# JiuTongBro/vqnerf_release

Measured on AMD Instinct MI355X. Metric: rays/sec (render) 800x800, 64+64 samples/ray, NeuS SDF 8x256 + colour 4x256, higher is better.
Workload: dtype f32; 1 GPU; BASELINE configs[1], nerf/hotdog-shaped NeuS render: one whole 800x800 pin-hole view per rank per step (camera at distance 4, fov 0.6911), n_samples=64, n_importance=64, up_sample_steps=4, sdf 8x256; parallelism=views x1 (no data-path collective)

## Files before the change

include/vqn_neus_fold.h:

```cpp
#ifndef VQN_NEUS_FOLD_H_
#define VQN_NEUS_FOLD_H_
#include <stdint.h>
#ifdef __cplusplus
extern "C" {
#endif

int64_t vqn_neus_fold_pack(const int32_t* sdf_desc, const int32_t* col_desc, const float* wbuf_col, int64_t col_floats,
                           const float* sdf_w_last, const float* sdf_b_last, int sdf_hidden, int d_feature, const float* col_w0,
                           const float* col_b0, int col_hidden, float* wbuf_out, int64_t out_floats, int32_t* col_desc_out,
                           void* stream);

int vqn_mc_classify(const float* u, int nx, int ny, int nz, float threshold, int32_t* vert_count, int32_t* tri_count, void* stream);
int vqn_mc_emit(const float* u, int nx, int ny, int nz, float threshold, const int32_t* vert_offset, const int32_t* tri_offset,
                int64_t n_verts, int64_t n_tris, const float* origin, const float* step, float* verts, int32_t* tris, void* stream);

int vqn_mesh_components(const int32_t* tris, int64_t n_tris, int64_t n_verts, int32_t* labels, void* stream);
int vqn_mesh_remap_tris(const int32_t* tris_in, int64_t n_tris, const uint8_t* keep_tri, const int32_t* tri_offset,
                        const int32_t* new_index, int64_t n_verts, int32_t* tris_out, int64_t n_out, void* stream);

int vqn_mc_brick_points(const float* ax, const float* ay, const float* az, int nx, int ny, int nz, const int32_t* brick_ijk,
                        int64_t n_bricks, int64_t first, int64_t count, float* pts, void* stream);
int vqn_mc_brick_classify(const float* ub, const int32_t* brick_ijk, int64_t n_bricks, const int32_t* slot, int nx, int ny, int nz,
                          float threshold, int32_t* vert_count, int32_t* tri_count, int64_t* keys, int32_t* leaks, void* stream);
int vqn_mc_brick_emit(const float* ub, const int32_t* brick_ijk, int64_t n_bricks, const int32_t* slot, int nx, int ny, int nz,
                      float threshold, const int32_t* vert_offset, const int32_t* tri_offset, int64_t n_verts, int64_t n_tris,
                      const float* origin, const float* step, float* verts, int32_t* tris, void* stream);

int64_t vqn_image_metrics_scratch_bytes(int64_t B, int H, int W);
int vqn_image_metrics_u8(const uint8_t* a, const uint8_t* b, const float* alpha, int64_t alpha_stride, float alpha_thres, int64_t B,
                         int H, int W, int C, const double* window, void* scratch, int64_t scratch_bytes, void* out, void* stream);
int vqn_image_metrics_f32(const float* a, const float* b, const float* alpha, int64_t alpha_stride, float alpha_thres, int64_t B,
                          int H, int W, int C, const double* window, void* scratch, int64_t scratch_bytes, void* out, void* stream);

int64_t vqn_seg_scratch_bytes(int64_t n, int R, int C);
int vqn_seg_contingency_rgb(const uint8_t* gt_rgb, const uint8_t* pd_rgb, const float* alpha, float alpha_thres, int64_t n,
                            const uint8_t* gt_palette, int n_gt, const uint8_t* pd_palette, int n_pd, void* scratch,
                            int64_t scratch_bytes, void* out, void* stream);
int vqn_seg_contingency_labels(const int32_t* gt, const int32_t* pd, const uint8_t* mask, int64_t n, int n_gt, int n_pd,
                               void* scratch, int64_t scratch_bytes, void* out, void* stream);

int vqn_meanshift_seek(const double* points, int64_t n, const double* seeds, int64_t n_seeds, int D, double bandwidth, int max_iter,
                       double* means, int32_t* counts, int32_t* iters, void* stream);
int64_t vqn_meanshift_merge_scratch_bytes(int64_t n_candidates, int D);
int vqn_meanshift_merge(const double* candidates, const int32_t* cand_counts, int64_t n_candidates, int D, double bandwidth,
                        void* scratch, int64_t scratch_bytes, uint8_t* kept, int32_t* n_kept, void* stream);
int vqn_meanshift_assign(const double* points, int64_t n, const double* centres, int K, int D, double bandwidth, int32_t* labels,
                         double* dist, void* stream);

#ifdef __cplusplus
}
#endif
#endif
```

vqnerf_release_amd/_C.py:

```python
import contextlib
import ctypes
import os
import re

import numpy as np
import torch

_HERE = os.path.dirname(os.path.abspath(__file__))
LIB_PATH = os.environ.get('VQN_LIB', os.path.join(_HERE, 'lib', 'libvqnerf_hip.so'))
_lib = None

_ABI = """
i vqn_version()  s vqn_last_error()  i vqn_vq_assign(plipipppppp)  i vqn_vq_assign_variant(iiii)  i vqn_vq_ema_stats(ppliippplp)
l vqn_vq_ema_stats_ws_bytes(lii)  i vqn_vq_ste_loss(pplfpppp)  i vqn_vq_ema_update(pppiidfpppppppp)
i vqn_decomp_loss_fwd(ppppppliiffffffpp)  i vqn_decomp_loss_bwd(ppppppliiffffffpppppp)  i vqn_l2_normalize_rows(plifpp)
i vqn_l2_normalize_rows_bwd(pplifpp)  i vqn_vq_ste_loss_bwd(pppplpp)  i vqn_codebook_prep(ppiifpp)  i vqn_sim_smooth_fwd(piifpp)
i vqn_sim_smooth_bwd(pppiifpp)  i vqn_vq_quantize_rows(plipipffpppppp)  i vqn_vq_train_bwd(pppppflifpp)
i vqn_vq_quantize_rows_train(plipipfffppppppp)  i vqn_mlp_chain_fwd(ppplpipipipip)  i vqn_mlp_chain_fwd_f16s(ppplpipipipip)
i vqn_brdf_shade_fwd(pppppppliippppppppppppipipp)  i vqn_brdf_shade_fwd_rows(ppppppppliippppppppppppipipp)
l vqn_brdf_shade_bwd_partials(l)  i vqn_brdf_shade_bwd(pppppppliipppppppppppppppp)  i vqn_neus_sdf_points(pppppplipp)
l vqn_neus_fine_scratch_bytes(p)  i vqn_neus_fine_points(pppppppppliplpppp)  i vqn_neus_train_fwd(pppppplplpiiiipppp)
l vqn_neus_train_bwd_scratch_bytes(p)  i vqn_neus_train_bwd(ppppppplplpipip)  l vqn_neus_train_bwd_x3_scratch_bytes(p)
i vqn_neus_train_bwd_x3(pppppppplplpipip)  i vqn_pack_x3_gather(pplpp)  i vqn_pack_x3_gather2(pplpplpp)
i vqn_neus_sdf_points_f16s(pppppplipp)  i vqn_neus_fine_points_f16s(pppppppppliplpppp)  i vqn_neus_sdf_points_x3(pppppplipp)
i vqn_neus_fine_points_x3(pppppppppliplpppp)  i vqn_neus_train_fwd_x3(pppppplplpiiiipppp)  i vqn_neus_pack_create(piiifiiiiiip)
i vqn_neus_pack_update(pppppp)  p vqn_neus_pack_sdf_desc(p)  p vqn_neus_pack_col_desc(p)  p vqn_neus_pack_sdf_wbuf(p)
p vqn_neus_pack_col_wbuf(p)  l vqn_neus_pack_sdf_floats(p)  l vqn_neus_pack_col_floats(p)  v vqn_neus_pack_destroy(p)
l vqn_neus_sdf_pack_plan(piiifiiippl)  l vqn_neus_col_pack_plan(iiiiiiiiippl)  i vqn_mlp_chain_vq_fwd(ppppplpppppiffpppppp)
i vqn_vq_codebook_frags(piipp)  i vqn_linear2srgb(plpp)  i vqn_chain_pack_create(iiiipp)  i vqn_chain_pack_update(pppp)
i vqn_chain_pack_n_weights(p)  p vqn_chain_pack_desc(p)  p vqn_chain_pack_wbuf(p)  l vqn_chain_pack_floats(p)
v vqn_chain_pack_destroy(p)  l vqn_chain_pack_plan(iiiipppl)  i vqn_neus_upsample(ppppliffpipp)  i vqn_neus_merge(ppppliippp)
i vqn_neus_section_mids(plifpppp)  i vqn_neus_composite_fwd(pppppppppliffppppppppppp)  i vqn_neus_composite_bwd(pppppppppliffpppppppppp)
i vqn_tile_program(pppppilp)  l vqn_tile_program_grid(pl)  i vqn_weight_norm_fwd(ipppppp)  i vqn_weight_norm_bwd(ipppppppp)
i vqn_tfmt_pack(plilpip)  i vqn_tfmt_pack_delta(plilpipip)  i vqn_tfmt_unpack(piliplp)  i vqn_wgrad_partials(piiipiiilippp)
i vqn_wgrad_partials_x3(piiipiiilippp)  i vqn_wgrad_partials_batched(ipppppppplippip)  i vqn_reduce_partials(piiiplip)
i vqn_wgrad_finalize(ipppppppppppppp)  i vqn_clip_preserve(plffpp)  i vqn_loss_total(plppiiipp)  i vqn_ks_split_fwd(ppilppp)
i vqn_ks_split_bwd(ppilppppp)  i vqn_wgrad_thin_batched(ippppppppplippp)  i vqn_multi_copy(ipppp)  i vqn_refl_train_desc_ints()
i vqn_refl_train_fwd_x3(ppppplpippiip)  i vqn_refl_train_fwd_x3_zx(pppppplpipppiip)  l vqn_refl_train_bwd_x3_scratch_bytes(p)
i vqn_refl_train_bwd_x3(ppplpppipipippiiiplp)  i vqn_adam_step(ippppppppdddddiip)
"""
ABI = {name: (ret, args) for ret, name, args in re.findall(r'(\w) (\w+)\((\w*)\)', _ABI)}
ABI_FOLD = {'vqn_neus_fold_pack': ('l', 'ppplppiippiplpp'), 'vqn_mc_classify': ('i', 'piiifppp'), 'vqn_mc_emit': ('i', 'piiifppllppppp'),
            'vqn_mesh_components': ('i', 'pllpp'), 'vqn_mesh_remap_tris': ('i', 'plppplplp'),
            'vqn_mc_brick_points': ('i', 'pppiiiplllpp'), 'vqn_mc_brick_classify': ('i', 'pplpiiifppppp'),
            'vqn_mc_brick_emit': ('i', 'pplpiiifppllppppp'), 'vqn_image_metrics_scratch_bytes': ('l', 'lii'),
            'vqn_image_metrics_u8': ('i', 'ppplfliiipplpp'), 'vqn_image_metrics_f32': ('i', 'ppplfliiipplpp'),
            'vqn_seg_scratch_bytes': ('l', 'lii'), 'vqn_seg_contingency_rgb': ('i', 'pppflpipiplpp'),
            'vqn_seg_contingency_labels': ('i', 'pppliiplpp'), 'vqn_meanshift_seek': ('i', 'plplidipppp'),
            'vqn_meanshift_merge_scratch_bytes': ('l', 'li'), 'vqn_meanshift_merge': ('i', 'pplidplppp'),
            'vqn_meanshift_assign': ('i', 'plpiidppp')}
_CTYPES = dict(p=ctypes.c_void_p, i=ctypes.c_int, l=ctypes.c_int64, f=ctypes.c_float, d=ctypes.c_double, s=ctypes.c_char_p, v=None)


class VqnError(RuntimeError):
    pass


def build(verbose=False):
    import subprocess
    cmd = ['make', '-C', os.path.join(_HERE, 'csrc'), '-j8']
    if not verbose:
        cmd.append('-s')
    subprocess.check_call(cmd)


def lib():
    global _lib
    if _lib is None:
        if not os.path.exists(LIB_PATH):
            raise VqnError(f'{LIB_PATH} is missing: run `python -c "import __graft_entry__ as g; g.build()"` '
                           '(or `make -C vqnerf_release_amd/csrc`). There is no non-HIP fallback.')
        L = ctypes.CDLL(LIB_PATH)
        for name, (ret, args) in list(ABI.items()) + list(ABI_FOLD.items()):
            f = getattr(L, name)
            f.restype, f.argtypes = _CTYPES[ret], [_CTYPES[a] for a in args]
        _lib = L
    return _lib


def require_device(t, what):
    if not t.is_cuda:
        raise VqnError(f'{what}: got a {t.device} tensor; the no-graph path runs on MI355X HIP kernels only '
                       '(there is no CPU fallback)')
    lib()


def _check(rc, name, count=False):
    if (rc > 0) if count else (rc == 0):
        return rc
    raise VqnError(f'{name} failed (rc={rc or -3}): {lib().vqn_last_error().decode()}')


def _call(name, *args, clock=True, count=False):
    with _clock(name if clock is True else clock) if clock else contextlib.nullcontext():
        rc = getattr(lib(), name)(*args, _stream())
    return _check(rc, name, count)


def _ptr(t):
    return t if t is None or isinstance(t, int) else t.data_ptr()


def _ptrs(ts, n=1):
    return (ctypes.c_void_p * max(n, len(ts)))(*[_ptr(t) for t in ts])


def _host(a, dtype=np.int32):
    return np.ascontiguousarray(a, dtype=dtype).ctypes


def _i32(desc):
    d = np.ascontiguousarray(desc, dtype=np.int32)
    return d, d.ctypes.data_as(ctypes.c_void_p)


def _stream():
    return torch.cuda.current_stream().cuda_stream


class KernelClock:
    enabled = False
    pairs = {}
    _free = []

    @classmethod
# ... 184 lines not shown
    if g_ste is not None:
        _f32c(g_ste, 'g_ste')
    gz = torch.empty_like(z)
    _call('vqn_vq_train_bwd', _ptr(z), _ptr(xnorm), _ptr(quant), _ptr(g_ste), _ptr(g_loss), loss_post, z.shape[0], z.shape[1], eps, _ptr(gz))
    return gz


def l2_normalize_rows(x, eps=1e-6):
    _f32c(x, 'x')
    y = torch.empty_like(x)
    _call('vqn_l2_normalize_rows', _ptr(x), x.shape[0], x.shape[1], eps, _ptr(y))
    return y


def vq_quantize_rows(z, codebook, sel_mask=None, eps=1e-6, want_ste=True, want_xnorm=False, loss_post=1.0):
    _f32c(z, 'z'); _f32c(codebook, 'codebook')
    N, D = z.shape
    K = codebook.shape[1]
    assert codebook.shape[0] == D
    dev = z.device
    idx = torch.empty((N,), dtype=torch.int64, device=dev)
    ste = torch.empty((N, D), dtype=torch.float32, device=dev) if want_ste else None
    loss = torch.empty((), dtype=torch.float32, device=dev)
    counts = torch.empty((K,), dtype=torch.float32, device=dev)
    ws = torch.empty((4096,), dtype=torch.float32, device=dev)
    if sel_mask is not None:
        sel_mask = _f32c(sel_mask.reshape(-1).to(torch.float32).contiguous(), 'sel_mask')
        assert sel_mask.numel() == K
    n = N * D
    if want_xnorm:
        xnorm = torch.empty((N, D), dtype=torch.float32, device=dev)
        _call('vqn_vq_quantize_rows_train', _ptr(z), N, D, _ptr(codebook), K, _ptr(sel_mask), eps, 1.0 / n if n else 0.0, loss_post, _ptr(ws),
              _ptr(idx), _ptr(ste), _ptr(loss), _ptr(counts), _ptr(xnorm))
        return idx, ste, loss, counts, xnorm
    _call('vqn_vq_quantize_rows', _ptr(z), N, D, _ptr(codebook), K, _ptr(sel_mask), eps, 1.0 / n if n else 0.0, _ptr(ws), _ptr(idx), _ptr(ste),
          _ptr(loss), _ptr(counts))
    return idx, ste, loss, counts


_scratch_cache = {}
_scratch_held = []


def _scratch(tag, need, device, stream=None, capturing=None):
    if stream is None:
        stream = torch.cuda.current_stream().cuda_stream
    if capturing is None:
        capturing = torch.cuda.is_current_stream_capturing()
    key = (str(device), stream, tag)
    entry = _scratch_cache.get(key)
    if entry is None or entry[0].numel() < need:
        if entry is not None and entry[1]:
            _scratch_held.append(entry[0])
        entry = _scratch_cache[key] = [torch.empty((need,), dtype=torch.uint8, device=device), False]
    entry[1] = entry[1] or capturing
    return entry[0]


def _scratch_bytes(name, desc):
    need = getattr(lib(), name)(desc)
    if need <= 0:
        raise VqnError(f'{name}: invalid descriptor')
    return need


def neus_sdf_points(sdf_desc, wbuf_sdf, rays_o=None, rays_d=None, z=None, pts=None, mode='f32', pack=None):
    if pack is not None:
        dp, wp = pack.sdf_desc, pack.sdf_wbuf
    else:
        _f32c(wbuf_sdf, 'wbuf_sdf')
        dp, wp = _host(sdf_desc), _ptr(wbuf_sdf)
    if pts is not None:
        _f32c(pts, 'pts'); P, S = pts.shape[0], 1
        dev = pts.device
    else:
        _f32c(rays_o, 'rays_o'); _f32c(rays_d, 'rays_d'); _f32c(z, 'z')
        B, S = z.shape
        P = B * S
        dev = z.device
    out = torch.empty((P,), dtype=torch.float32, device=dev)
    entry = {'f32': 'vqn_neus_sdf_points', 'f16s': 'vqn_neus_sdf_points_f16s', 'x3': 'vqn_neus_sdf_points_x3'}[mode]
    _call(entry, dp, wp, _ptr(rays_o), _ptr(rays_d), _ptr(z), _ptr(pts), P, S, _ptr(out))
    return out


def neus_fine_points(sdf_desc, wbuf_sdf, col_desc, wbuf_col, rays_o=None, rays_d=None, z=None, pts=None, dirs=None, mode='f32'):
    _f32c(wbuf_sdf, 'wbuf_sdf'); _f32c(wbuf_col, 'wbuf_col')
    sdp, cdp = _host(sdf_desc), _host(col_desc)
    if pts is not None:
        _f32c(pts, 'pts'); _f32c(dirs, 'dirs'); P, S = pts.shape[0], 1
        dev = pts.device
    else:
        _f32c(rays_o, 'rays_o'); _f32c(rays_d, 'rays_d'); _f32c(z, 'z')
        B, S = z.shape
        P = B * S
        dev = z.device
    buf = _scratch('fine', _scratch_bytes('vqn_neus_fine_scratch_bytes', sdp), dev)
    sdf = torch.empty((P,), dtype=torch.float32, device=dev)
    grad = torch.empty((P, 3), dtype=torch.float32, device=dev)
    rgb = torch.empty((P, 3), dtype=torch.float32, device=dev)
    entry = {'f32': 'vqn_neus_fine_points', 'f16s': 'vqn_neus_fine_points_f16s', 'x3': 'vqn_neus_fine_points_x3'}[mode]
    _call(entry, sdp, _ptr(wbuf_sdf), cdp, _ptr(wbuf_col), _ptr(rays_o), _ptr(rays_d), _ptr(z), _ptr(pts), _ptr(dirs), P, S, _ptr(buf),
          buf.numel(), _ptr(sdf), _ptr(grad), _ptr(rgb))
    return sdf, grad, rgb


def neus_fold_pack(sdf_desc, col_desc, wbuf_col, sdf_w_last, sdf_b_last, col_w0, col_b0):
    for t in (wbuf_col, sdf_w_last, sdf_b_last, col_w0, col_b0):
        _f32c(t, 'weight / bias')
    (F1, H), C = sdf_w_last.shape, col_w0.shape[0]
    sdp, cdp = _host(sdf_desc), _host(col_desc)
    desc = np.zeros(len(col_desc), np.int32)
    args = (sdp, cdp, _ptr(wbuf_col), wbuf_col.numel(), _ptr(sdf_w_last), _ptr(sdf_b_last), H, F1 - 1, _ptr(col_w0), _ptr(col_b0), C)
    n = _call('vqn_neus_fold_pack', *args, None, 0, None, clock=False, count=True)
    out = torch.empty((n,), dtype=torch.float32, device=wbuf_col.device)
    _call('vqn_neus_fold_pack', *args, _ptr(out), n, desc.ctypes.data_as(ctypes.c_void_p), count=True)
    return out, desc


class NeusPackHandle:

    def __init__(self, sdf_dims, sdf_skip, multires, scale, col_mode, col_d_hidden, col_n_layers, multires_view, squeeze_out, engine):
        L = lib()
        self.h = ctypes.c_void_p()
        _check(L.vqn_neus_pack_create(_host(sdf_dims), len(sdf_dims) - 1, sdf_skip, multires, scale, col_mode, col_d_hidden, col_n_layers,
                                      multires_view, int(squeeze_out), engine, ctypes.byref(self.h)), 'vqn_neus_pack_create')
        self.sdf_desc, self.col_desc = L.vqn_neus_pack_sdf_desc(self.h), L.vqn_neus_pack_col_desc(self.h)
        self.sdf_wbuf, self.col_wbuf = L.vqn_neus_pack_sdf_wbuf(self.h), L.vqn_neus_pack_col_wbuf(self.h)

    def update(self, W, b, Wc, bc):
        for t in W + b + Wc + bc:
            _f32c(t, 'weight / bias')
        _call('vqn_neus_pack_update', self.h, _ptrs(W), _ptrs(b), _ptrs(Wc), _ptrs(bc))

    def __del__(self):
        try:
            if self.h:
                lib().vqn_neus_pack_destroy(self.h)
        except Exception:
            pass


def neus_train_fwd(sdf_desc, wbuf_sdf, col_desc, wbuf_col, pts, dirs, saved, e_tiles, outf_tiles, extr_tiles, out_sdf, out_n, out_rgb, pack=None):
    _f32c(pts, 'pts'); _f32c(dirs, 'dirs')
    for t in saved + [out_sdf, out_n, out_rgb]:
        _f32c(t, 'saved tensor')
    if pack is not None:
        sdp, cdp, wsp, wcp, entry = pack.sdf_desc, pack.col_desc, pack.sdf_wbuf, pack.col_wbuf, 'vqn_neus_train_fwd_x3'
    else:
        _f32c(wbuf_sdf, 'wbuf_sdf'); _f32c(wbuf_col, 'wbuf_col')
        sdp, cdp, wsp, wcp, entry = _host(sdf_desc), _host(col_desc), _ptr(wbuf_sdf), _ptr(wbuf_col), 'vqn_neus_train_fwd'
    P, dev = pts.shape[0], pts.device
    buf = _scratch('fine', _scratch_bytes('vqn_neus_fine_scratch_bytes', sdp), dev)
    _call(entry, sdp, wsp, cdp, wcp, _ptr(pts), _ptr(dirs), P, _ptr(buf), buf.numel(), _ptrs(saved), len(saved), e_tiles, outf_tiles,
          extr_tiles, _ptr(out_sdf), _ptr(out_n), _ptr(out_rgb))


def pack_x3_gather(flat, gidx, n_steps, fidx=None):
    _f32c(flat, 'flat')
    if gidx.dtype != torch.int32 or not gidx.is_contiguous() or gidx.numel() != n_steps * 512:
        raise VqnError('pack_x3_gather: gidx must be a contiguous int32 tensor of n_steps * 512 entries')
    out = torch.empty((n_steps, 3, 64, 8), dtype=torch.int16, device=flat.device)
    if fidx is None:
        _call('vqn_pack_x3_gather', _ptr(flat), _ptr(gidx), n_steps, _ptr(out))
        return out
    if fidx.dtype != torch.int32 or not fidx.is_contiguous() or fidx.device != flat.device:
# ... 587 lines not shown
```

vqnerf_release_amd/csrc/mlp_prims.h:

```cpp
#pragma once
#include "common.h"

namespace eng {

enum Act : int { ACT_NONE = 0, ACT_RELU = 1, ACT_SOFTPLUS100 = 2, ACT_SIGMOID = 3 };

__device__ __forceinline__ float fast_exp(float x) { return __builtin_amdgcn_exp2f(x * 1.4426950408889634f); }
__device__ __forceinline__ float fast_log(float x) { return __builtin_amdgcn_logf(x) * 0.6931471805599453f; }
__device__ __forceinline__ float fast_rcp(float x) { return __builtin_amdgcn_rcpf(x); }

template <int ACT>
__device__ __forceinline__ float act_fwd(float x) {
  if (ACT == ACT_RELU) return fmaxf(x, 0.f);
  if (ACT == ACT_SOFTPLUS100) {
    const float t = 100.f * x;
    return t > 20.f ? x : 0.01f * fast_log(1.f + fast_exp(t));
  }
  if (ACT == ACT_SIGMOID) return fast_rcp(1.f + fast_exp(-x));
  return x;
}

template <int ACT>
__device__ __forceinline__ float act_bwd_from_out(float h) {
  if (ACT == ACT_RELU) return h > 0.f ? 1.f : 0.f;
// ... 189 lines not shown
#pragma unroll
    for (int i = 0; i < 4; ++i) {
      if (first) a0[i] = pre[i]; else a0[i] = wp[min(i, ng - 1) * 64];
    }
    { const int r = brow(0); pc = lds[r]; qc = lds[r + img_stride]; }
    __builtin_amdgcn_s_waitcnt(0x0F70);
    init(ot, 0, acc0);
    init(ot, 1, acc1);
    __builtin_amdgcn_s_setprio(1);
    auto block = [&](const f32x4 (&a)[4], int g0) {
#pragma unroll
      for (int i = 0; i < 4; ++i) {
        { const int r = brow(g0 + i + 1); pn = lds[r]; qn = lds[r + img_stride]; }
        if (g0 + i < ng) {
#pragma unroll
          for (int j = 0; j < 4; ++j) {
            acc0 = __builtin_amdgcn_mfma_f32_32x32x2f32(a[i][j], pc[j], acc0, 0, 0, 0);
            acc1 = __builtin_amdgcn_mfma_f32_32x32x2f32(a[i][j], qc[j], acc1, 0, 0, 0);
          }
        }
        pc = pn; qc = qn;
      }
    };
    if ((ng & 7) == 0) {
      for (int g = 0; g < ng - 8; g += 8) {
#pragma unroll
        for (int i = 0; i < 4; ++i) a1[i] = wp[(g + 4 + i) * 64];
        block(a0, g);
#pragma unroll
        for (int i = 0; i < 4; ++i) a0[i] = wp[(g + 8 + i) * 64];
        block(a1, g + 4);
      }
#pragma unroll
      for (int i = 0; i < 4; ++i) a1[i] = wp[(ng - 4 + i) * 64];
      block(a0, ng - 8);
      if (use_pre && ot + NW >= n_out_tiles && next_wp != nullptr) {
#pragma unroll
        for (int i = 0; i < 4; ++i) pre[i] = next_wp[i * 64];
      }
      f32x4 qt[4];
#pragma unroll
      for (int i = 0; i < 4; ++i) {
        { const int r = brow(ng - 4 + i + 1); pn = lds[r]; qn = lds[r + img_stride]; }
        qt[i] = qc;
#pragma unroll
        for (int j = 0; j < 4; ++j) acc0 = __builtin_amdgcn_mfma_f32_32x32x2f32(a1[i][j], pc[j], acc0, 0, 0, 0);
        pc = pn; qc = qn;
      }
#pragma unroll
      for (int i = 0; i < 4; ++i) {
#pragma unroll
        for (int j = 0; j < 4; ++j) acc1 = __builtin_amdgcn_mfma_f32_32x32x2f32(a1[i][j], qt[i][j], acc1, 0, 0, 0);
        epi_rq(ot, 0, i, acc0);
      }
      __builtin_amdgcn_s_setprio(0);
#pragma unroll
      for (int rq = 0; rq < 4; ++rq) epi_rq(ot, 1, rq, acc1);
      continue;
    }
    for (int g = 0; g < ng; g += 8) {
#pragma unroll
      for (int i = 0; i < 4; ++i) a1[i] = wp[min(g + 4 + i, ng - 1) * 64];
      block(a0, g);
#pragma unroll
      for (int i = 0; i < 4; ++i) a0[i] = wp[min(g + 8 + i, ng - 1) * 64];
      block(a1, g + 4);
    }
    if (use_pre && ot + NW >= n_out_tiles && next_wp != nullptr) {
#pragma unroll
      for (int i = 0; i < 4; ++i) pre[i] = next_wp[i * 64];
    }
#pragma unroll
    for (int rq = 0; rq < 4; ++rq) epi_rq(ot, 0, rq, acc0);
    __builtin_amdgcn_s_setprio(0);
#pragma unroll
    for (int rq = 0; rq < 4; ++rq) epi_rq(ot, 1, rq, acc1);
  }
  if (use_pre && wave >= n_out_tiles && next_wp != nullptr) {
#pragma unroll
    for (int i = 0; i < 4; ++i) pre[i] = next_wp[i * 64];
  }
}

__device__ __forceinline__ f32x4 acc_quad(const f32x16& acc, int rq) {
  return (f32x4){acc[4 * rq + 0], acc[4 * rq + 1], acc[4 * rq + 2], acc[4 * rq + 3]};
}

__device__ __forceinline__ void init_bias(const f32x4* __restrict__ bpack, int ot, int lane, f32x16& acc) {
  const f32x4* b = bpack + ot * 8;
  const bool hi = lane >= 32;
#pragma unroll
  for (int rq = 0; rq < 4; ++rq) {
    const f32x4 v0 = b[rq], v1 = b[4 + rq];
    acc[4 * rq + 0] = hi ? v1[0] : v0[0]; acc[4 * rq + 1] = hi ? v1[1] : v0[1];
    acc[4 * rq + 2] = hi ? v1[2] : v0[2]; acc[4 * rq + 3] = hi ? v1[3] : v0[3];
  }
}

__device__ __forceinline__ void init_zero(f32x16& acc) {
#pragma unroll
  for (int i = 0; i < 16; ++i) acc[i] = 0.f;
}

__device__ __forceinline__ void init_rows(const f32x4* __restrict__ rows , int lane, f32x16& acc) {
#pragma unroll
  for (int rq = 0; rq < 4; ++rq) {
    f32x4 v = rows[rq * 64 + lane];
    acc[4 * rq + 0] = v[0]; acc[4 * rq + 1] = v[1]; acc[4 * rq + 2] = v[2]; acc[4 * rq + 3] = v[3];
  }
}

__device__ __forceinline__ float posenc_feat(int f, float x0, float x1, float x2) {
  if (f < 3) return f == 0 ? x0 : (f == 1 ? x1 : x2);
  const int g = f - 3, k = g / 6, m = g - 6 * k, c = m >= 3 ? m - 3 : m;
  const float xc = c == 0 ? x0 : (c == 1 ? x1 : x2);
  const float arg = xc * (float)(1 << k);
  return m < 3 ? sinf(arg) : cosf(arg);
}
__device__ __forceinline__ float posenc_jac(int f, float x0, float x1, float x2, int* comp) {
  if (f < 3) { *comp = f; return 1.f; }
  const int g = f - 3, k = g / 6, m = g - 6 * k, c = m >= 3 ? m - 3 : m;
  const float xc = c == 0 ? x0 : (c == 1 ? x1 : x2);
  const float fr = (float)(1 << k), arg = xc * fr;
  *comp = c;
  return m < 3 ? fr * cosf(arg) : -fr * sinf(arg);
}

__device__ __forceinline__ int row_feat(int r, int h, int j) { return 32 * (r >> 2) + 2 * (4 * (r & 3) + j) + h; }
__device__ __forceinline__ float lds_feat(const f32x4* __restrict__ lds, const int row0, const int f, const int pp) {
  const int t = f >> 5, fi = f & 31, hh = fi & 1, rr = fi >> 1;
  return reinterpret_cast<const float*>(lds)[(((row0 + t * 4 + (rr >> 2)) * 64) + pp + 32 * hh) * 4 + (rr & 3)];
}

template <int NOUT, int NW = 4>
__device__ __forceinline__ void rowdot(const f32x4* __restrict__ lds, int row0, int n_rows,
                                       const f32x4* __restrict__ wimg , float* out_s,
                                       int wave, int lane) {
  constexpr int CH = NOUT == 1 ? 8 : (NOUT <= 2 ? 4 : 3);
  float s[NOUT];
#pragma unroll
  for (int o = 0; o < NOUT; ++o) s[o] = 0.f;
  const int h = lane >> 5;
  for (int r0 = wave; r0 < n_rows; r0 += NW * CH) {
    f32x4 b[CH], wv[CH][NOUT];
#pragma unroll
    for (int c = 0; c < CH; ++c) {
      const int r = min(r0 + NW * c, n_rows - 1);
      b[c] = lds[(row0 + r) * 64 + lane];
#pragma unroll
      for (int o = 0; o < NOUT; ++o) wv[c][o] = wimg[(o * n_rows + r) * 2 + h];
    }
#pragma unroll
    for (int c = 0; c < CH; ++c)
      if (r0 + NW * c < n_rows) {
#pragma unroll
        for (int o = 0; o < NOUT; ++o) {
          s[o] = fmaf(b[c][0], wv[c][o][0], s[o]); s[o] = fmaf(b[c][1], wv[c][o][1], s[o]);
          s[o] = fmaf(b[c][2], wv[c][o][2], s[o]); s[o] = fmaf(b[c][3], wv[c][o][3], s[o]);
        }
      }
  }
#pragma unroll
  for (int o = 0; o < NOUT; ++o) {
    s[o] += __shfl_xor(s[o], 32);
    if (h == 0) out_s[(wave * 32 + (lane & 31)) * NOUT + o] = s[o];
  }
// ... 4 lines not shown
```

vqnerf_release_amd/csrc/neus_launch.h:

```cpp
#pragma once
#include "neus_phases.h"


static int neus_sdf_args(const char* fn, const int32_t* sdf_desc, const float* wbuf_sdf, const float* rays_o, const float* rays_d,
                         const float* z, const float* pts, const int64_t P, const int S, const float* out_sdf,
                         int (*check_desc)(const SdfDesc&), const char* desc_msg, SdfDesc* sd) {
  VQN_CHECK_ARG_IN(fn, sdf_desc && wbuf_sdf && out_sdf, "sdf_desc, wbuf_sdf, out_sdf must be non-null");
  VQN_CHECK_ARG_IN(fn, P >= 0, "P >= 0");
  if (P == 0) return VQN_OK;
  VQN_CHECK_ARG_IN(fn, pts != nullptr || (rays_o && rays_d && z && S > 0), "either pts or (rays_o, rays_d, z, S) required");
  memcpy(sd, sdf_desc, sizeof(SdfDesc));
  VQN_CHECK_SHAPE_IN(fn, check_desc(*sd) == 0, desc_msg);
  return VQN_OK;
}

static int neus_fine_args(const char* fn, const int32_t* sdf_desc, const float* wbuf_sdf, const int32_t* col_desc, const float* wbuf_col,
                          const float* rays_o, const float* rays_d, const float* z, const float* pts, const float* dirs, const int64_t P,
                          const int S, const void* scratch, const float* out_sdf, const float* out_grad, const float* out_rgb,
                          int (*check_desc)(const SdfDesc&), const char* desc_msg, bool (*extras_rows_ok)(const ColDesc&),
                          SdfDesc* sd, ColDesc* cd) {
  VQN_CHECK_ARG_IN(fn, sdf_desc && wbuf_sdf && col_desc && wbuf_col, "descriptors and weight packs must be non-null");
  VQN_CHECK_ARG_IN(fn, out_sdf && out_grad && scratch, "out_sdf, out_grad and scratch must be non-null");
  VQN_CHECK_ARG_IN(fn, P >= 0, "P >= 0");
  if (P == 0) return VQN_OK;
  VQN_CHECK_ARG_IN(fn, (pts != nullptr && dirs != nullptr) || (rays_o && rays_d && z && S > 0),
                   "either (pts, dirs) or (rays_o, rays_d, z, S) required");
  memcpy(sd, sdf_desc, sizeof(SdfDesc));
  memcpy(cd, col_desc, sizeof(ColDesc));
  VQN_CHECK_SHAPE_IN(fn, check_desc(*sd) == 0, desc_msg);
  if (cd->n_lin != 0) {
    VQN_CHECK_ARG_IN(fn, out_rgb != nullptr, "out_rgb must be non-null when a colour net is given");
    VQN_CHECK_SHAPE_IN(fn, sd->layers[sd->n_lin - 1].n_out_tiles >= 1, "SDF network has no feature outputs (d_out == 1)");
    VQN_CHECK_SHAPE_IN(fn, cd->n_lin >= 2 && cd->n_lin <= VQN_MAX_COL_LAYERS && cd->d_out == 3, "colour net: 2..8 layers, d_out == 3");
    VQN_CHECK_SHAPE_IN(fn, cd->extra_feats >= 3 && cd->extra_feats <= 64 && extras_rows_ok(*cd), "colour net extras");
    for (int l = 0; l < cd->n_lin - 1; ++l)
      VQN_CHECK_SHAPE_IN(fn, cd->layers[l].n_out_tiles >= 1 && cd->layers[l].n_out_tiles <= sd->max_tiles, "colour layer wider than max_tiles");
  }
  return VQN_OK;
}

static eng::TrainOut neus_train_out(float* const* tensors, const int nL, const int nC, const int e_tiles, const int outf_tiles, const int extr_tiles) {
  eng::TrainOut to;
  memset(&to, 0, sizeof(to));
  to.E = tensors[0]; to.OUTF = tensors[1]; to.EXTR = tensors[2];
  for (int l = 1; l <= nL; ++l) to.U[l] = tensors[3 + (l - 1)];
  for (int l = 0; l < nL; ++l) to.GH[l] = tensors[3 + nL + l];
  for (int l = 1; l <= nC; ++l) to.C[l] = tensors[3 + 2 * nL + (l - 1)];
  to.e_tiles = e_tiles; to.outf_tiles = outf_tiles; to.extr_tiles = extr_tiles;
  return to;
}

static int64_t neus_stash_bytes(const SdfDesc& sd) { return (int64_t)(sd.n_lin - 1) * 4 * sd.max_tiles * 1024; }

static long pair_grid(const long n_tiles, const int images, const int64_t per_img, const int64_t scratch_bytes) {
  long grid = (long)vqn_num_cus() * (images == 1 ? 2 : 1);
  const long groups = (n_tiles + images - 1) / images;
  if (grid > groups) grid = groups;
  if ((int64_t)grid * images * per_img > scratch_bytes) grid = (long)(scratch_bytes / (images * per_img));
  return grid;
}

template <class Kernel, class... Args>
static int neus_launch(const char* fn, const Kernel kernel, const bool opt_in, const long grid, const int threads, const size_t lds, void* stream,
                       const Args... args) {
  if (opt_in) VQN_HIP_IN(fn, hipFuncSetAttribute((const void*)kernel, hipFuncAttributeMaxDynamicSharedMemorySize, (int)lds));
  hipLaunchKernelGGL(kernel, dim3((unsigned)grid), dim3(threads), lds, (hipStream_t)stream, args...);
  VQN_HIP_IN(fn, hipGetLastError());
  return VQN_OK;
}
```

vqnerf_release_amd/csrc/neus_mlp.hip:

```cpp
#include "neus_launch.h"
#include <stdlib.h>

using namespace eng;

#ifdef VQN_STAMPS
__device__ unsigned long long g_stamps[8];
#define VQN_STAMP_DECL unsigned long long st_[6] = {0, 0, 0, 0, 0, 0}; unsigned long long st_prev = __builtin_amdgcn_s_memtime(); const unsigned long long st_begin = st_prev;
#define VQN_STAMP(i) { const unsigned long long st_now = __builtin_amdgcn_s_memtime(); st_[i] += st_now - st_prev; st_prev = st_now; }
#define VQN_STAMP_FLUSH if (threadIdx.x == 0) { st_[5] = __builtin_amdgcn_s_memtime() - st_begin; for (int i_ = 0; i_ < 6; ++i_) atomicAdd(&g_stamps[i_], st_[i_]); atomicAdd(&g_stamps[6], 1ull); }
extern "C" int vqn_debug_read_stamps(unsigned long long* out, int reset) {
  if (hipMemcpyFromSymbol(out, HIP_SYMBOL(g_stamps), sizeof(unsigned long long) * 8) != hipSuccess) return -3;
  if (reset) { unsigned long long z[8] = {0, 0, 0, 0, 0, 0, 0, 0}; if (hipMemcpyToSymbol(HIP_SYMBOL(g_stamps), z, sizeof(z)) != hipSuccess) return -3; }
  return 0;
}
#else
#define VQN_STAMP_DECL
#define VQN_STAMP(i)
#define VQN_STAMP_FLUSH
#endif

#ifdef VQN_STAMPS
__device__ unsigned long long g_stamps2[16];
#define FS_DECL unsigned long long fs_[16] = {0, 0, 0, 0, 0, 0, 0, 0, 0, 0, 0, 0, 0, 0, 0, 0}; unsigned long long fs_prev = __builtin_amdgcn_s_memtime(); const unsigned long long fs_begin = fs_prev;
#define FS(i) { const unsigned long long fs_now = __builtin_amdgcn_s_memtime(); fs_[i] += fs_now - fs_prev; fs_prev = fs_now; }
// ... 471 lines not shown
      const float px = sm->pts[img][p * 3 + 0], py = sm->pts[img][p * 3 + 1], pz = sm->pts[img][p * 3 + 2];
      const float dx = sm->dirs[img][p * 3 + 0], dy = sm->dirs[img][p * 3 + 1], dz = sm->dirs[img][p * 3 + 2];
      for (int r = w4; r < (TRAIN ? 4 * to.extr_tiles : cd.extra_rows); r += 4) {
        f32x4 v;
#pragma unroll
        for (int j = 0; j < 4; ++j)
          v[j] = r < cd.extra_rows ? col_extra_feat(row_feat(r, h, j), px, py, pz, dx, dy, dz, sm->grad[img] + p * 3, cd.n_view_feats, cd.extra_feats) : 0.f;
        if (r < cd.extra_rows) ldsi[(E0 + r) * 64 + lane] = v;
        if (TRAIN && ptile_w < n_tiles) tfmt_store_quad(to.EXTR, ptile_w, to.extr_tiles, r >> 2, r & 3, lane, v);
      }
      const f32x4* sv = save0 + (size_t)img * per_img + (size_t)feat_slot * 64;
      const int feat_rows = 4 * sd.layers[n_lin - 1].n_out_tiles;
      for (int r0 = w4; r0 < (fold ? 0 : feat_rows); r0 += 32) {
        f32x4 v[8];
#pragma unroll
        for (int c = 0; c < 8; ++c) v[c] = ld_stream(sv + min(r0 + 4 * c, feat_rows - 1) * 64 + lane);
#pragma unroll
        for (int c = 0; c < 8; ++c)
          if (r0 + 4 * c < feat_rows) ldsi[(X0 + r0 + 4 * c) * 64 + lane] = v[c];
      }
      __syncthreads();
      FS(10)
      cur = X0; oth = Y0;
      int in_rows = feat_rows;
      if (fold) {
        const LayerDesc L = cd.layers[0];
        const int dst = oth;
        gemm_tiles2<8>(lds, IS, KSegs{E0, cd.extra_rows, 0, 0}, wcol + cd.reserved3, L.n_out_tiles, wave, lane, nopre, false, nullptr,
                       [&](int ot, int im, f32x16& acc) {
                         const f32x4* pp = save0 + (size_t)im * per_img + (size_t)feat_slot * 64 + ot * 256 + lane;
#pragma unroll
                         for (int rq = 0; rq < 4; ++rq) {
                           const f32x4 v = ld_stream(pp + rq * 64);
                           acc[4 * rq + 0] = v[0]; acc[4 * rq + 1] = v[1]; acc[4 * rq + 2] = v[2]; acc[4 * rq + 3] = v[3];
                         }
                       },
                       [&](int ot, int im, int rq, const f32x16& acc) {
                         f32x4* li = lds + (size_t)im * IS;
                         f32x4 v = {acc[4 * rq], acc[4 * rq + 1], acc[4 * rq + 2], acc[4 * rq + 3]};
#pragma unroll
                         for (int j = 0; j < 4; ++j) v[j] = act_fwd<ACT_RELU>(v[j]);
                         li[(dst + ot * 4 + rq) * 64 + lane] = v;
                       });
        __syncthreads();
        const int t = cur; cur = oth; oth = t;
        in_rows = 4 * L.n_out_tiles;
      }
      for (int l = fold ? 1 : 0; l < cd.n_lin - 1; ++l) {
        const LayerDesc L = cd.layers[l];
        const KSegs ks{cur, in_rows, E0, l == 0 ? cd.extra_rows : 0};
        const f32x4* bp = wcol + L.b_off;
        const int dst = oth;
        float* const t_c = TRAIN ? to.C[l + 1] : nullptr;
        gemm_tiles2<8>(lds, IS, ks, wcol + L.w_off, L.n_out_tiles, wave, lane, nopre, false, nullptr,
                       [&](int ot, int, f32x16& acc) { init_bias(bp, ot, lane, acc); },
                       [&](int ot, int im, int rq, const f32x16& acc) {
                         f32x4* li = lds + (size_t)im * IS;
                         f32x4 v = {acc[4 * rq], acc[4 * rq + 1], acc[4 * rq + 2], acc[4 * rq + 3]};
#pragma unroll
                         for (int j = 0; j < 4; ++j) v[j] = act_fwd<ACT_RELU>(v[j]);
                         li[(dst + ot * 4 + rq) * 64 + lane] = v;
                         if (TRAIN && 2 * pair + im < n_tiles) tfmt_store_quad(t_c, 2 * pair + im, L.n_out_tiles, ot, rq, lane, v);
                       });
        __syncthreads();
        const int t = cur; cur = oth; oth = t;
        in_rows = 4 * L.n_out_tiles;
      }
      FS(11)
      rowdot<3>(ldsi, cur, in_rows, wcol + cd.last_w_off, sm->part[img], w4, lane);
      __syncthreads();
      if (tid < 192) {
        const int im = tid / 96, r = tid - 96 * im, pp = r & 31, o = r >> 5;
        const float v = rgb_out(sm->part[im], pp, o, cd.last_b_off, cd.last_bias[o], cd.squeeze_out, wcol);
        const long pt = ((2 * pair + im) << 5) + pp;
        if (pt < P) out_rgb[pt * 3 + o] = v;
      }
    }
    __syncthreads();
  }
  FS(12)
  FS_FLUSH
}

int check_sdf_desc(const SdfDesc& d) {
  if (d.n_lin < 2 || d.n_lin > VQN_MAX_SDF_LAYERS) return 1;
  if (d.max_tiles < 1 || d.max_tiles > 16) return 2;
  if (d.emb_feats < 3 || d.emb_feats > 64 || d.emb_rows < 1 || d.emb_rows > 8) return 3;
  if (d.skip >= d.n_lin - 1 || d.skip == 0) return 4;
  for (int l = 0; l < d.n_lin; ++l)
    if (d.layers[l].n_out_tiles < 0 || d.layers[l].n_out_tiles > d.max_tiles) return 5;
  if (!(d.scale > 0.f)) return 6;
  return 0;
}

template <int NIMG>
size_t lds_bytes(int MT) { return (size_t)NIMG * (E_ROWS + 8 * MT) * 1024 + sizeof(Smalls<NIMG>); }

bool use_two_images(int MT) {
  static const bool forced32 = getenv("VQN_NEUS_TILE32") != nullptr;
  return !forced32 && MT >= 5 && lds_bytes<2>(MT) <= 160 * 1024;
}

bool extras_rows_ok(const ColDesc& cd) { return cd.extra_rows >= 1 && cd.extra_rows <= 8; }

}

extern "C" int vqn_neus_sdf_points(const int32_t* sdf_desc, const float* wbuf_sdf, const float* rays_o,
                                   const float* rays_d, const float* z, const float* pts, int64_t P, int S,
                                   float* out_sdf, void* stream) {
  SdfDesc sd;
  const int rc = neus_sdf_args(__func__, sdf_desc, wbuf_sdf, rays_o, rays_d, z, pts, P, S, out_sdf, check_sdf_desc,
                               "invalid SDF network descriptor", &sd);
  if (rc != VQN_OK || P == 0) return rc;
  ColDesc cd;
  memset(&cd, 0, sizeof(cd));
  const long n_tiles = (P + 31) / 32;
  const f32x4* ws = reinterpret_cast<const f32x4*>(wbuf_sdf);
  if (use_two_images(sd.max_tiles))
    return neus_launch(__func__, neus_points2_kernel<false>, true, pair_grid(n_tiles, 2, 0, 0), 512, lds_bytes<2>(sd.max_tiles), stream, sd, cd, ws,
                       nullptr, rays_o, rays_d, z, pts, nullptr, (long)P, S, nullptr, out_sdf, nullptr, nullptr, TrainOut{});
  const size_t lds = lds_bytes<1>(sd.max_tiles);
  VQN_CHECK_SHAPE(lds <= 160 * 1024, "network too wide for LDS");
  return neus_launch(__func__, neus_points_kernel<false>, lds > 64 * 1024, pair_grid(n_tiles, 1, 0, 0), 256, lds, stream, sd, cd, ws, nullptr, rays_o, rays_d,
                     z, pts, nullptr, (long)P, S, nullptr, out_sdf, nullptr, nullptr);
}

extern "C" int vqn_neus_train_fwd(const int32_t* sdf_desc, const float* wbuf_sdf, const int32_t* col_desc, const float* wbuf_col,
                                  const float* pts, const float* dirs, int64_t P, void* scratch, int64_t scratch_bytes,
                                  float* const* tensors, int n_tensors, int e_tiles, int outf_tiles, int extr_tiles, float* out_sdf,
                                  float* out_n, float* out_rgb, void* stream) {
  VQN_CHECK_ARG(sdf_desc && wbuf_sdf && col_desc && wbuf_col && pts && dirs && scratch && tensors && out_sdf && out_n && out_rgb, "null pointer");
  VQN_CHECK_ARG(P >= 1, "P >= 1");
  SdfDesc sd;
  ColDesc cd;
  memcpy(&sd, sdf_desc, sizeof(SdfDesc));
  memcpy(&cd, col_desc, sizeof(ColDesc));
  VQN_CHECK_SHAPE(check_sdf_desc(sd) == 0, "invalid SDF network descriptor");
  VQN_CHECK_SHAPE(cd.n_lin >= 2 && cd.n_lin <= VQN_MAX_COL_LAYERS && cd.d_out == 3 && sd.layers[sd.n_lin - 1].n_out_tiles >= 1, "colour net");
  VQN_CHECK_SHAPE(use_two_images(sd.max_tiles), "the training forward kernel is the two-image form only");
  const int nL = sd.n_lin - 1, nC = cd.n_lin - 1;
  VQN_CHECK_ARG(n_tensors == 3 + 2 * nL + nC, "tensors: [E, OUTF, EXTR, U_1..U_nL, GH_0..GH_{nL-1}, C_1..C_nC]");
  VQN_CHECK_SHAPE(e_tiles * 4 >= sd.emb_rows && e_tiles <= 2 && extr_tiles * 4 >= cd.extra_rows && extr_tiles <= 2 &&
                  outf_tiles >= sd.layers[sd.n_lin - 1].n_out_tiles, "tile counts");
  for (int i = 0; i < n_tensors; ++i) VQN_CHECK_ARG(tensors[i] != nullptr, "null tensor pointer");
  const long grid = pair_grid((P + 31) / 32, 2, neus_stash_bytes(sd), scratch_bytes);
  VQN_CHECK_ARG(grid >= 1, "scratch too small (see vqn_neus_fine_scratch_bytes)");
  return neus_launch(__func__, neus_points2_kernel<true, true>, true, grid, 512, lds_bytes<2>(sd.max_tiles), stream, sd, cd,
                     reinterpret_cast<const f32x4*>(wbuf_sdf), reinterpret_cast<const f32x4*>(wbuf_col), nullptr, nullptr, nullptr, pts, dirs,
                     (long)P, 1, reinterpret_cast<f32x4*>(scratch), out_sdf, out_n, out_rgb,
                     neus_train_out(tensors, nL, nC, e_tiles, outf_tiles, extr_tiles));
}

extern "C" int64_t vqn_neus_fine_scratch_bytes(const int32_t* sdf_desc) {
  if (!sdf_desc) return -1;
  SdfDesc sd;
  memcpy(&sd, sdf_desc, sizeof(SdfDesc));
  const int emb_rows = sd.emb_rows;
  if (emb_rows >= 1 && emb_rows <= 12) sd.emb_rows = 1;
  if (check_sdf_desc(sd) != 0) return -2;
#ifdef VQN_DIAG_STASH_ROT
  return (int64_t)VQN_DIAG_STASH_ROT * vqn_num_cus() * 2 * neus_stash_bytes(sd);
#else
  return (int64_t)vqn_num_cus() * 2 * neus_stash_bytes(sd);
#endif
}

extern "C" int vqn_neus_fine_points(const int32_t* sdf_desc, const float* wbuf_sdf, const int32_t* col_desc,
                                    const float* wbuf_col, const float* rays_o, const float* rays_d, const float* z,
                                    const float* pts, const float* dirs, int64_t P, int S, void* scratch,
                                    int64_t scratch_bytes, float* out_sdf, float* out_grad, float* out_rgb,
                                    void* stream) {
  SdfDesc sd;
  ColDesc cd;
  const int rc = neus_fine_args(__func__, sdf_desc, wbuf_sdf, col_desc, wbuf_col, rays_o, rays_d, z, pts, dirs, P, S, scratch, out_sdf,
                                out_grad, out_rgb, check_sdf_desc, "invalid SDF network descriptor", extras_rows_ok, &sd, &cd);
  if (rc != VQN_OK || P == 0) return rc;
  if (cd.n_lin != 0)
    VQN_CHECK_ARG((cd.reserved1 > 0 && cd.reserved2 > cd.reserved1 && cd.reserved3 > cd.reserved2) ||
                  (cd.reserved1 == 0 && cd.reserved2 == 0 && cd.reserved3 == 0), "col_desc: fold offsets (reserved1..3) inconsistent");
  const long n_tiles = (P + 31) / 32;
  const int64_t per_img = neus_stash_bytes(sd);
  const f32x4* ws = reinterpret_cast<const f32x4*>(wbuf_sdf);
  const f32x4* wc = reinterpret_cast<const f32x4*>(wbuf_col);
  if (use_two_images(sd.max_tiles)) {
    const bool fold = cd.n_lin != 0 && cd.reserved1 > 0;
#ifdef VQN_DIAG_STASH_ROT
    const long grid = pair_grid(n_tiles, 2, 0, 0);
    VQN_CHECK_ARG((int64_t)VQN_DIAG_STASH_ROT * grid * 2 * per_img <= scratch_bytes, "diag build: scratch must hold ROT regions per workgroup");
#else
    const long grid = pair_grid(n_tiles, 2, per_img, scratch_bytes);
#endif
    VQN_CHECK_ARG(grid >= 1, "scratch too small (see vqn_neus_fine_scratch_bytes)");
    return neus_launch(__func__, fold ? neus_points2_kernel<true, false, true> : neus_points2_kernel<true>, true, grid, 512, lds_bytes<2>(sd.max_tiles),
                       stream, sd, cd, ws, wc, rays_o, rays_d, z, pts, dirs, (long)P, S, reinterpret_cast<f32x4*>(scratch), out_sdf, out_grad,
                       out_rgb, TrainOut{});
  }
  const size_t lds = lds_bytes<1>(sd.max_tiles);
  VQN_CHECK_SHAPE(lds <= 160 * 1024, "network too wide for LDS");
  const long grid = pair_grid(n_tiles, 1, per_img, scratch_bytes);
  VQN_CHECK_ARG(grid >= 1, "scratch too small (see vqn_neus_fine_scratch_bytes)");
  return neus_launch(__func__, neus_points_kernel<true>, lds > 64 * 1024, grid, 256, lds, stream, sd, cd, ws, wc, rays_o, rays_d, z, pts, dirs, (long)P, S,
                     reinterpret_cast<f32x4*>(scratch), out_sdf, out_grad, out_rgb);
}
```

Baseline: 281,100 rays/s.

## Add two-workgroup-per-CU paired-tile SDF kernel with in-place MFMA layers

Adds a new SDF-only kernel that processes two 32-point tiles per 256-thread workgroup. Each wave computes up to two output tiles per layer in place in LDS, prefetches the next layer's weights, and raises wave priority around the MFMA loop. Because it uses less LDS than the lockstep 512-thread form, two workgroups can fit per CU. A new selector picks this form when max_tiles<=8, LDS<=80KB and the occupancy query allows two blocks, and a query API exposes the choice. The trade-off is an extra barrier per layer and duplicated weight reads across the co-resident workgroups.

```diff
diff --git a/include/vqn_neus_fold.h b/include/vqn_neus_fold.h
--- a/include/vqn_neus_fold.h
+++ b/include/vqn_neus_fold.h
@@ -9,6 +9,8 @@
                            const float* sdf_w_last, const float* sdf_b_last, int sdf_hidden, int d_feature, const float* col_w0,
                            const float* col_b0, int col_hidden, float* wbuf_out, int64_t out_floats, int32_t* col_desc_out,
                            void* stream);
+
+int vqn_neus_sdf_form(const int32_t* sdf_desc, int32_t* out);
 
 int vqn_mc_classify(const float* u, int nx, int ny, int nz, float threshold, int32_t* vert_count, int32_t* tri_count, void* stream);
 int vqn_mc_emit(const float* u, int nx, int ny, int nz, float threshold, const int32_t* vert_offset, const int32_t* tri_offset,
diff --git a/vqnerf_release_amd/_C.py b/vqnerf_release_amd/_C.py
--- a/vqnerf_release_amd/_C.py
+++ b/vqnerf_release_amd/_C.py
@@ -40,7 +40,7 @@
 i vqn_refl_train_bwd_x3(ppplpppipipippiiiplp)  i vqn_adam_step(ippppppppdddddiip)
 """
 ABI = {name: (ret, args) for ret, name, args in re.findall(r'(\w) (\w+)\((\w*)\)', _ABI)}
-ABI_FOLD = {'vqn_neus_fold_pack': ('l', 'ppplppiippiplpp'), 'vqn_mc_classify': ('i', 'piiifppp'), 'vqn_mc_emit': ('i', 'piiifppllppppp'),
+ABI_FOLD = {'vqn_neus_fold_pack': ('l', 'ppplppiippiplpp'), 'vqn_neus_sdf_form': ('i', 'pp'), 'vqn_mc_classify': ('i', 'piiifppp'), 'vqn_mc_emit': ('i', 'piiifppllppppp'),
             'vqn_mesh_components': ('i', 'pllpp'), 'vqn_mesh_remap_tris': ('i', 'plppplplp'),
             'vqn_mc_brick_points': ('i', 'pppiiiplllpp'), 'vqn_mc_brick_classify': ('i', 'pplpiiifppppp'),
             'vqn_mc_brick_emit': ('i', 'pplpiiifppllppppp'), 'vqn_image_metrics_scratch_bytes': ('l', 'lii'),
@@ -391,6 +391,12 @@
     entry = {'f32': 'vqn_neus_sdf_points', 'f16s': 'vqn_neus_sdf_points_f16s', 'x3': 'vqn_neus_sdf_points_x3'}[mode]
     _call(entry, dp, wp, _ptr(rays_o), _ptr(rays_d), _ptr(z), _ptr(pts), P, S, _ptr(out))
     return out
+
+
+def neus_sdf_form(sdf_desc):
+    out = np.zeros(3, np.int32)
+    _check(lib().vqn_neus_sdf_form(_host(sdf_desc), out.ctypes), 'vqn_neus_sdf_form')
+    return {'form': ('tile32', 'lockstep', 'pairs')[int(out[0])], 'lds_bytes': int(out[1]), 'wgs_per_cu': int(out[2])}
 
 
 def neus_fine_points(sdf_desc, wbuf_sdf, col_desc, wbuf_col, rays_o=None, rays_d=None, z=None, pts=None, dirs=None, mode='f32'):
diff --git a/vqnerf_release_amd/csrc/mlp_prims.h b/vqnerf_release_amd/csrc/mlp_prims.h
--- a/vqnerf_release_amd/csrc/mlp_prims.h
+++ b/vqnerf_release_amd/csrc/mlp_prims.h
@@ -295,6 +295,102 @@
   }
 }
 
+__device__ __forceinline__ void init_bias(const f32x4* __restrict__ bpack, int ot, int lane, f32x16& acc);
+template <int ACT>
+__device__ __forceinline__ void gemm_layer2_inplace(f32x4* __restrict__ lds, const int img_stride, const KSegs ks, const int dst_row,
+                                                    const f32x4* __restrict__ w, const f32x4* __restrict__ bpack,
+                                                    const int n_out_tiles, const int wave, const int lane, f32x4 (&pre)[4],
+                                                    const f32x4* __restrict__ next_wp) {
+  const int ng = ks.nA + ks.nB;
+  const bool hasA = wave < n_out_tiles, hasB = wave + 4 < n_out_tiles;
+  f32x16 accA0, accA1, accB0, accB1;
+  auto act16 = [&](f32x16& acc) {
+#pragma unroll
+    for (int k = 0; k < 16; ++k) acc[k] = act_fwd<ACT>(acc[k]);
+  };
+  if (hasA) {
+    auto brow = [&](int g) { g = g < ng ? g : 0; return ((g < ks.nA) ? (ks.rowA + g) : (ks.rowB + (g - ks.nA))) * 64 + lane; };
+    const f32x4* __restrict__ wpA = w + (size_t)wave * ng * 64 + lane;
+    const f32x4* __restrict__ wpB = w + (size_t)(hasB ? wave + 4 : wave) * ng * 64 + lane;
+    f32x4 a0[4], a1[4], pc, qc, pn, qn;
+    auto group = [&](const f32x4& af, f32x16& c0, f32x16& c1) {
+#pragma unroll
+      for (int j = 0; j < 4; ++j) {
+        c0 = __builtin_amdgcn_mfma_f32_32x32x2f32(af[j], pc[j], c0, 0, 0, 0);
+        c1 = __builtin_amdgcn_mfma_f32_32x32x2f32(af[j], qc[j], c1, 0, 0, 0);
+      }
+    };
+    auto block = [&](const f32x4 (&a)[4], int g0, f32x16& c0, f32x16& c1) {
+#pragma unroll
+      for (int i = 0; i < 4; ++i) {
+        { const int r = brow(g0 + i + 1); pn = lds[r]; qn = lds[r + img_stride]; }
+        if (g0 + i < ng) group(a[i], c0, c1);
+        pc = pn; qc = qn;
+      }
+    };
+    auto fill = [&](const f32x4* __restrict__ wp, f32x4 (&a)[4], int g0) {
+#pragma unroll
+      for (int i = 0; i < 4; ++i) a[i] = wp[min(g0 + i, ng - 1) * 64];
+    };
+#pragma unroll
+    for (int i = 0; i < 4; ++i) a0[i] = pre[i];
+    { const int r = brow(0); pc = lds[r]; qc = lds[r + img_stride]; }
+    __builtin_amdgcn_s_waitcnt(0x0F70);
+    init_bias(bpack, wave, lane, accA0);
+    accA1 = accA0;
+    __builtin_amdgcn_s_setprio(1);
+    for (int g = 0; g < ng; g += 8) {
+      fill(wpA, a1, g + 4);
+      block(a0, g, accA0, accA1);
+      if (g + 8 < ng) fill(wpA, a0, g + 8); else fill(wpB, a0, 0);
+      block(a1, g + 4, accA0, accA1);
+    }
+    if (hasB) {
+      init_bias(bpack, wave + 4, lane, accB0);
+      accB1 = accB0;
+      fill(wpB, a1, 4);
+#pragma unroll
+      for (int i = 0; i < 4; ++i) {
+        { const int r = brow(i + 1); pn = lds[r]; qn = lds[r + img_stride]; }
+        if (i < ng) group(a0[i], accB0, accB1);
+        pc = pn; qc = qn;
+#pragma unroll
+        for (int j = 0; j < 4; ++j) {
+          accA0[4 * i + j] = act_fwd<ACT>(accA0[4 * i + j]);
+          accA1[4 * i + j] = act_fwd<ACT>(accA1[4 * i + j]);
+        }
+      }
+      fill(wpB, a0, 8);
+      block(a1, 4, accB0, accB1);
+      for (int g = 8; g < ng; g += 8) {
+        fill(wpB, a1, g + 4);
+        block(a0, g, accB0, accB1);
+        fill(wpB, a0, g + 8);
+        block(a1, g + 4, accB0, accB1);
+      }
+    }
+    __builtin_amdgcn_s_setprio(0);
+  }
+  if (next_wp != nullptr) {
+#pragma unroll
+    for (int i = 0; i < 4; ++i) pre[i] = next_wp[i * 64];
+  }
+  if (hasB) { act16(accB0); act16(accB1); }
+  else if (hasA) { act16(accA0); act16(accA1); }
+  __syncthreads();
+  auto put = [&](const int ot, const f32x16& c0, const f32x16& c1) {
+#pragma unroll
+    for (int rq = 0; rq < 4; ++rq) {
+      const int r = (dst_row + ot * 4 + rq) * 64 + lane;
+      lds[r] = (f32x4){c0[4 * rq], c0[4 * rq + 1], c0[4 * rq + 2], c0[4 * rq + 3]};
+      lds[r + img_stride] = (f32x4){c1[4 * rq], c1[4 * rq + 1], c1[4 * rq + 2], c1[4 * rq + 3]};
+    }
+  };
+  if (hasA) put(wave, accA0, accA1);
+  if (hasB) put(wave + 4, accB0, accB1);
+  __syncthreads();
+}
+
 __device__ __forceinline__ f32x4 acc_quad(const f32x16& acc, int rq) {
   return (f32x4){acc[4 * rq + 0], acc[4 * rq + 1], acc[4 * rq + 2], acc[4 * rq + 3]};
 }
diff --git a/vqnerf_release_amd/csrc/neus_launch.h b/vqnerf_release_amd/csrc/neus_launch.h
--- a/vqnerf_release_amd/csrc/neus_launch.h
+++ b/vqnerf_release_amd/csrc/neus_launch.h
@@ -52,8 +52,8 @@
 
 static int64_t neus_stash_bytes(const SdfDesc& sd) { return (int64_t)(sd.n_lin - 1) * 4 * sd.max_tiles * 1024; }
 
-static long pair_grid(const long n_tiles, const int images, const int64_t per_img, const int64_t scratch_bytes) {
-  long grid = (long)vqn_num_cus() * (images == 1 ? 2 : 1);
+static long pair_grid(const long n_tiles, const int images, const int64_t per_img, const int64_t scratch_bytes, const int wgs_per_cu = 0) {
+  long grid = (long)vqn_num_cus() * (wgs_per_cu > 0 ? wgs_per_cu : (images == 1 ? 2 : 1));
   const long groups = (n_tiles + images - 1) / images;
   if (grid > groups) grid = groups;
   if ((int64_t)grid * images * per_img > scratch_bytes) grid = (long)(scratch_bytes / (images * per_img));
diff --git a/vqnerf_release_amd/csrc/neus_mlp.hip b/vqnerf_release_amd/csrc/neus_mlp.hip
--- a/vqnerf_release_amd/csrc/neus_mlp.hip
+++ b/vqnerf_release_amd/csrc/neus_mlp.hip
@@ -577,6 +577,68 @@
   FS_FLUSH
 }
 
+struct SdfPairSmalls {
+  float pts[2][96], part[2][128];
+};
+
+__global__ __launch_bounds__(256, 2) void neus_sdf_pairs_kernel(
+    const SdfDesc sd, const f32x4* __restrict__ wsdf, const float* __restrict__ rays_o, const float* __restrict__ rays_d,
+    const float* __restrict__ zv, const float* __restrict__ pts_direct, const long P, const int S, float* __restrict__ out_sdf) {
+  extern __shared__ __attribute__((aligned(16))) f32x4 lds[];
+  const int ER = sd.emb_rows, IS = (ER + 4 * sd.max_tiles) * 64;
+  const int X0 = ER;
+  SdfPairSmalls* sm = reinterpret_cast<SdfPairSmalls*>(lds + (size_t)2 * IS);
+  const int tid = threadIdx.x, lane = tid & 63, h = lane >> 5, p = lane & 31;
+  const int wave = __builtin_amdgcn_readfirstlane(tid >> 6);
+  const int n_lin = sd.n_lin;
+  const long n_tiles = (P + 31) >> 5, n_pairs = (n_tiles + 1) >> 1;
+  f32x4 pre[4];
+
+  for (long pair = blockIdx.x; pair < n_pairs; pair += gridDim.x) {
+    if (tid < 64) {
+      const int im = tid >> 5, t = tid & 31;
+      float no_dirs[3];
+      load_point<false>(((2 * pair + im) << 5) + t, P, S, rays_o, rays_d, zv, pts_direct, nullptr, sm->pts[im] + t * 3, no_dirs);
+    }
+    __syncthreads();
+    for (int r = wave; r < ER; r += 4) {
+#pragma unroll
+      for (int im = 0; im < 2; ++im) {
+        const float xs = sm->pts[im][p * 3 + 0] * sd.scale, ys = sm->pts[im][p * 3 + 1] * sd.scale, zs = sm->pts[im][p * 3 + 2] * sd.scale;
+        f32x4 v;
+#pragma unroll
+        for (int j = 0; j < 4; ++j) v[j] = emb_feat(row_feat(r, h, j), sd.emb_feats, xs, ys, zs);
+        lds[im * IS + (E0 + r) * 64 + lane] = v;
+      }
+    }
+    if (wave < sd.layers[0].n_out_tiles) {
+      const f32x4* wp0 = wsdf + sd.layers[0].w_off + (size_t)wave * ER * 64 + lane;
+#pragma unroll
+      for (int i = 0; i < 4; ++i) pre[i] = wp0[min(i, ER - 1) * 64];
+    }
+    __syncthreads();
+
+    for (int l = 0; l < n_lin - 1; ++l) {
+      const LayerDesc L = sd.layers[l];
+      const f32x4* next_wp = nullptr;
+      if (l + 1 < n_lin - 1 && wave < sd.layers[l + 1].n_out_tiles)
+        next_wp = wsdf + sd.layers[l + 1].w_off + (size_t)wave * (4 * L.n_out_tiles + ((l + 1 == sd.skip) ? ER : 0)) * 64 + lane;
+      const KSegs ks = (l == 0) ? KSegs{E0, ER, 0, 0} : KSegs{X0, 4 * sd.layers[l - 1].n_out_tiles, E0, (l == sd.skip) ? ER : 0};
+      gemm_layer2_inplace<ACT_SOFTPLUS100>(lds, IS, ks, X0, wsdf + L.w_off, wsdf + L.b_off, L.n_out_tiles, wave, lane, pre, next_wp);
+    }
+
+    const int hid_rows = 4 * sd.layers[n_lin - 2].n_out_tiles;
+#pragma unroll
+    for (int im = 0; im < 2; ++im) rowdot<1>(lds + (size_t)im * IS, X0, hid_rows, wsdf + sd.last_w_off, sm->part[im], wave, lane);
+    __syncthreads();
+    if (tid < 64) {
+      const int im = tid >> 5, t = tid & 31;
+      const long pt = ((2 * pair + im) << 5) + t;
+      if (pt < P) out_sdf[pt] = sdf_raw(sm->part[im], t, sd.last_b_off, sd.last_bias, wsdf) / sd.scale;
+    }
+  }
+}
+
 int check_sdf_desc(const SdfDesc& d) {
   if (d.n_lin < 2 || d.n_lin > VQN_MAX_SDF_LAYERS) return 1;
   if (d.max_tiles < 1 || d.max_tiles > 16) return 2;
@@ -594,6 +656,37 @@
 bool use_two_images(int MT) {
   static const bool forced32 = getenv("VQN_NEUS_TILE32") != nullptr;
   return !forced32 && MT >= 5 && lds_bytes<2>(MT) <= 160 * 1024;
+}
+
+enum SdfForm : int { SDF_FORM_TILE32 = 0, SDF_FORM_LOCKSTEP = 1, SDF_FORM_PAIRS = 2 };
+
+size_t lds_bytes_pairs(const SdfDesc& sd) { return (size_t)2 * (sd.emb_rows + 4 * sd.max_tiles) * 1024 + sizeof(SdfPairSmalls); }
+
+int sdf_pairs_wgs_per_cu(const size_t lds) {
+  static int known[81];
+  int& k = known[lds >> 10];
+  if (k == 0) {
+    int n = 0;
+    if (hipFuncSetAttribute((const void*)neus_sdf_pairs_kernel, hipFuncAttributeMaxDynamicSharedMemorySize, (int)lds) != hipSuccess ||
+        hipOccupancyMaxActiveBlocksPerMultiprocessor(&n, (const void*)neus_sdf_pairs_kernel, 256, lds) != hipSuccess) {
+      (void)hipGetLastError();
+      n = 0;
+    }
+    k = n + 1;
+  }
+  return k - 1;
+}
+
+SdfForm sdf_form(const SdfDesc& sd, size_t* lds, int* wgs_per_cu) {
+  const int MT = sd.max_tiles;
+  if (!use_two_images(MT)) { *lds = lds_bytes<1>(MT); *wgs_per_cu = 2; return SDF_FORM_TILE32; }
+  const size_t lp = lds_bytes_pairs(sd);
+  if (getenv("VQN_NEUS_SDF_LOCKSTEP") == nullptr && MT <= 8 && lp <= 80 * 1024) {
+    const int n = sdf_pairs_wgs_per_cu(lp);
+    if (n >= 2) { *lds = lp; *wgs_per_cu = 2; return SDF_FORM_PAIRS; }
+  }
+  *lds = lds_bytes<2>(MT); *wgs_per_cu = 1;
+  return SDF_FORM_LOCKSTEP;
 }
 
 bool extras_rows_ok(const ColDesc& cd) { return cd.extra_rows >= 1 && cd.extra_rows <= 8; }
@@ -611,13 +704,31 @@
   memset(&cd, 0, sizeof(cd));
   const long n_tiles = (P + 31) / 32;
   const f32x4* ws = reinterpret_cast<const f32x4*>(wbuf_sdf);
-  if (use_two_images(sd.max_tiles))
-    return neus_launch(__func__, neus_points2_kernel<false>, true, pair_grid(n_tiles, 2, 0, 0), 512, lds_bytes<2>(sd.max_tiles), stream, sd, cd, ws,
+  size_t lds;
+  int wgs;
+  const SdfForm form = sdf_form(sd, &lds, &wgs);
+  if (form == SDF_FORM_PAIRS)
+    return neus_launch(__func__, neus_sdf_pairs_kernel, true, pair_grid(n_tiles, 2, 0, 0, 2), 256, lds, stream, sd, ws, rays_o, rays_d, z, pts,
+                       (long)P, S, out_sdf);
+  if (form == SDF_FORM_LOCKSTEP)
+    return neus_launch(__func__, neus_points2_kernel<false>, true, pair_grid(n_tiles, 2, 0, 0), 512, lds, stream, sd, cd, ws,
                        nullptr, rays_o, rays_d, z, pts, nullptr, (long)P, S, nullptr, out_sdf, nullptr, nullptr, TrainOut{});
-  const size_t lds = lds_bytes<1>(sd.max_tiles);
   VQN_CHECK_SHAPE(lds <= 160 * 1024, "network too wide for LDS");
   return neus_launch(__func__, neus_points_kernel<false>, lds > 64 * 1024, pair_grid(n_tiles, 1, 0, 0), 256, lds, stream, sd, cd, ws, nullptr, rays_o, rays_d,
                      z, pts, nullptr, (long)P, S, nullptr, out_sdf, nullptr, nullptr);
+}
+
+extern "C" int vqn_neus_sdf_form(const int32_t* sdf_desc, int32_t* out) {
+  VQN_CHECK_ARG(sdf_desc && out, "null pointer");
+  SdfDesc sd;
+  memcpy(&sd, sdf_desc, sizeof(SdfDesc));
+  VQN_CHECK_SHAPE(check_sdf_desc(sd) == 0, "invalid SDF network descriptor");
+  size_t lds;
+  int wgs;
+  out[0] = (int32_t)sdf_form(sd, &lds, &wgs);
+  out[1] = (int32_t)lds;
+  out[2] = wgs;
+  return VQN_OK;
 }
 
 extern "C" int vqn_neus_train_fwd(const int32_t* sdf_desc, const float* wbuf_sdf, const int32_t* col_desc, const float* wbuf_col,
```

After: 282,900 rays/s, median of 6. About the same (+0.7%).
